# AsherBond/0-kno-vectorx

Measured on AMD Instinct MI355X. Metric: header_range_256 proofs/sec, higher is better.
Workload: dtype u64 (Goldilocks) / u8 (hashes)

## Files before the change

0-kno-vectorx_amd/csrc/vx_bus.hip:

```cpp
#include <string.h>

#include <memory>

#include "vx_bus.h"
#include "vx_table_shapes.h"

int32_t vx_one_table_hook(void*, const uint64_t* pub, size_t n_pub, const uint64_t* cap, size_t cw, uint64_t* chal, size_t n_chal) {
    vx_shared_challenges_n(&pub, &n_pub, &cap, 1, cw, chal, n_chal);
    return VX_OK;
}

int32_t vx_tables_proof_bound(const vx_stark_config* cfg, size_t hdr_words, const TableShape* tables, size_t n_tables, size_t* n_words) {
    size_t total = hdr_words;
    for (size_t k = 0; k < n_tables; ++k) {
        size_t w = 0;
        VX_TRY(vx_stark_proof_bound(tables[k].air_id, cfg, tables[k].log_n, &w));
        total += w;
    }
    *n_words = total;
    return VX_OK;
}
int32_t vx_tables_proof_bound(const vx_stark_config* cfg, size_t hdr_words, std::initializer_list<TableShape> tables, size_t* n_words) {
    return vx_tables_proof_bound(cfg, hdr_words, tables.begin(), tables.size(), n_words);
}
std::array<TableShape, 3> vx_justification_shapes(size_t n_authorities, size_t n_sig) {
    return {{{VX_AIR_SHA_CHAIN, sha_log_n(n_authorities)}, {ed_air_id(n_sig), ed_log_n(n_sig)}, {s512_air_id(n_sig), s512_log_n(n_sig)}}};
}
size_t vx_justification_proof_bound(const vx_stark_config* cfg, size_t n_authorities, int32_t* rc_out) {
    const auto sh = vx_justification_shapes(n_authorities, sig_quorum(n_authorities));
    size_t w = 0;
    *rc_out = vx_tables_proof_bound(cfg, 0, {sh[0], sh[1], sh[2]}, &w);
    return w;
}

static int32_t size_proof(TableJob& j, int air_id, int log_n, const vx_stark_config* cfg) {
    size_t bound = 0;
    VX_TRY(vx_stark_proof_bound(air_id, cfg, log_n, &bound));
    j.proof.resize(bound);
    return VX_OK;
}
int32_t run_table(vx_ctx* c, TableJob& j, int air_id, int log_n, size_t n_cols, size_t n_pub, const vx_stark_config* cfg, const vx_chal_hook* hook, int consume_trace,
                  const TableGen& gen) {
    VX_TRY(size_proof(j, air_id, log_n, cfg));
    vx_buf* trace = nullptr;
    VX_TRY(vx_alloc(c, n_cols << log_n, &trace));
    uint64_t pub[BusMeet::MAX_PUB];
    int32_t r = gen(c, trace, pub);
    if (r == VX_OK) r = vx_stark_prove_impl(c, air_id, cfg, trace->d, trace->n, consume_trace, log_n, pub, n_pub, j.proof.data(), j.proof.size(), &j.len, hook);
    (void)vx_free(c, trace);
    return r;
}
int TableGroup::add(TableSpec s, int bus, bool local) {
    const int k = g.add(bus, local);
    spec[k] = std::move(s);
    hook[k] = {vx_bus_hook, &g.t[k].party};
    return k;
}
int32_t TableGroup::contexts(int here) {
    if (have_contexts) return VX_OK;
    vx_ctx* c = ctx;
    for (int k = 0; k < g.n; ++k)
        if (g.local(k)) job[k].c = k == here ? ctx : (c = c ? vx_side_ctx(c) : nullptr);
    VX_CHECK(c, "%s: no side context for every table (the provers meet at their challenge hooks, each on a context of its own)", what);
    have_contexts = true;
    return VX_OK;
}
int32_t TableGroup::run(int k) {
    const TableSpec& s = spec[k];
    TableJob& j = job[k];
    if (s.gen) return run_table(j.c, j, s.air_id, s.log_n, s.n_cols, s.n_pub, cfg, &hook[k], s.consume_trace, s.gen);
    VX_TRY(size_proof(j, s.air_id, s.log_n, cfg));
    return vx_stark_prove_impl(j.c, s.air_id, cfg, s.trace->d, s.trace->n, s.consume_trace, s.log_n, s.pub, s.n_pub, j.proof.data(), j.proof.size(), &j.len, &hook[k]);
}
int32_t TableGroup::prove(int here, std::vector<int> order) {
    VX_TRY(contexts(here));
    for (int k = 0; k < g.n; ++k)
        if (g.local(k) && k != here) {
            job[k].c->err.clear();
            g.start(k, [this, k] {
                (void)hipSetDevice(job[k].c->device);
                return run(k);
            });
        }
    if (here >= 0) g.run_here(here, [&] { return run(here); });
    g.finish();
    if (order.empty()) {
        if (here >= 0) order.push_back(here);
        for (int k = 0; k < g.n; ++k)
            if (k != here) order.push_back(k);
    }
    int who = -1;
    const int32_t rc = g.first_error(order, &who);
    if (rc == VX_OK || (who >= 0 && who == here)) return rc;
    if (who < 0) return vx_fail(ctx, rc, "%s: %s", what, BusGroup::ALL_RELEASED);
    const char* msg = vx_last_error(job[who].c);
    if (!msg[0]) return vx_fail(ctx, rc, "%s: the %s table failed", what, spec[who].name);
    if (strncmp(msg, what, strlen(what)) == 0) return vx_fail(ctx, rc, "%s", msg);
    return vx_fail(ctx, rc, "%s: %s", what, msg);
}
int32_t pack_blob(vx_ctx* ctx, const char* what, uint64_t magic, const uint64_t* request, size_t n_request, const TableJob* const* jobs, size_t n_jobs, uint64_t* blob_out, size_t blob_cap,
                  size_t* blob_len) {
    size_t total = 1 + n_request + n_jobs;
    for (size_t k = 0; k < n_jobs; ++k) total += jobs[k]->len;
    *blob_len = total;
    if (!blob_out || blob_cap < total) return vx_fail(ctx, VX_ERR_BUFSZ, "%s: the blob needs %zu words, buffer has %zu", what, total, blob_cap);
    uint64_t* w = blob_out;
    *w++ = magic;
    for (size_t k = 0; k < n_request; ++k) *w++ = request[k];
    for (size_t k = 0; k < n_jobs; ++k) *w++ = jobs[k]->len;
    for (size_t k = 0; k < n_jobs; ++k) memcpy(w, jobs[k]->proof.data(), jobs[k]->len * 8), w += jobs[k]->len;
    return VX_OK;
}
int32_t pack_blob(vx_ctx* ctx, const char* what, uint64_t magic, std::initializer_list<uint64_t> request, std::initializer_list<const TableJob*> jobs, uint64_t* blob_out,
                  size_t blob_cap, size_t* blob_len) {
    return pack_blob(ctx, what, magic, request.begin(), request.size(), jobs.begin(), jobs.size(), blob_out, blob_cap, blob_len);
}

int vx_justification_add(TableGroup& g, const vx_justification* just, std::function<int32_t(vx_ctx*)> pre, int bus, unsigned mask) {
    const size_t n_auth = just->num_authorities;
    auto chosen = std::make_shared<std::vector<uint8_t>>(n_auth, 0);
    size_t n_sig = 0;
    for (size_t i = 0; i < n_auth && n_sig < sig_quorum(n_auth); ++i)
        if (just->validator_signed[i]) (*chosen)[i] = 1, ++n_sig;
    const auto sh = vx_justification_shapes(n_auth, n_sig);
    const int sl = sh[0].log_n, el = sh[1].log_n, hl = sh[2].log_n;
    const int first = g.add({"authority-set commitment", sh[0].air_id, sl, VX_SHA_AIR_COLS, 10, 0,
                             [=](vx_ctx* c, vx_buf* st, uint64_t* spub) {
                                 if (pre) VX_TRY(pre(c));
                                 uint8_t com[32];
                                 VX_TRY(vx_sha_chain_trace_dev(c, just->pubkeys, n_auth, chosen->data(), 1, sl, st->d, spub, com));
                                 if (memcmp(com, just->authority_set_hash, 32) != 0) return vx_fail(c, VX_ERR_STATEMENT, "authority-set commitment mismatch");
                                 return (int32_t)VX_OK;
                             }},
                            bus, mask & 1);
    g.add({"Ed25519", sh[1].air_id, el, VX_ED_AIR_COLS, 2, 0,
           [=](vx_ctx* c, vx_buf* et, uint64_t* epub) { return vx_ed_trace_dev(c, just->pubkeys, just->signatures, just->precommit, 53, chosen->data(), n_auth, el, 1, et->d, epub); }},
          bus, mask >> 1 & 1);
    g.add({"SHA-512", sh[2].air_id, hl, VX_SHA512_AIR_COLS, 15, 0,
           [=](vx_ctx* c, vx_buf* ht, uint64_t* hpub) { return vx_sha512_trace_dev(c, just->pubkeys, just->signatures, just->precommit, chosen->data(), n_auth, hl, 1, ht->d, hpub); }},
          bus, mask >> 2 & 1);
    return first;
}
```

0-kno-vectorx_amd/csrc/vx_core.hip:

```cpp
#include <stdarg.h>
#include <stdlib.h>
#include <stdio.h>

#include "gl.cuh"
#include <dlfcn.h>

#include "vx_internal.h"

__attribute__((constructor)) static void vx_runtime_env() { setenv("GPU_MAX_HW_QUEUES", "16", 0); }

int32_t vx_fail(vx_ctx* ctx, int32_t code, const char* fmt, ...) {
    char buf[512];
    va_list ap;
    va_start(ap, fmt);
    vsnprintf(buf, sizeof buf, fmt, ap);
    va_end(ap);
    if (ctx) ctx->err = buf;
    return code;
}

static int32_t make_powtab(vx_ctx* ctx, uint64_t base, PowTab* out) {
    std::vector<uint64_t> h(3 * 2048);
    uint64_t b = base;
    for (int l = 0; l < 3; ++l) {
        uint64_t acc = 1;
        for (int j = 0; j < 2048; ++j) {
            h[l * 2048 + j] = acc;
            acc = glh::mul(acc, b);
        }
        b = glh::pow(b, 2048);
    }
    VX_HIP(hipMalloc(&out->d, h.size() * 8));
    VX_HIP(hipMemcpyAsync(out->d, h.data(), h.size() * 8, hipMemcpyHostToDevice, ctx->stream));
    VX_HIP(hipStreamSynchronize(ctx->stream));
    return VX_OK;
}

int32_t vx_get_shift_tab(vx_ctx* ctx, uint64_t base, PowTab* out) {
    auto it = ctx->shift_tabs.find(base);
    if (it == ctx->shift_tabs.end()) {
        PowTab t;
        VX_TRY(make_powtab(ctx, base, &t));
        it = ctx->shift_tabs.emplace(base, t).first;
    }
    *out = it->second;
    return VX_OK;
}

int32_t vx_get_tw2(vx_ctx* ctx, int log_s, int inverse, Tw2* out) {
    const int lo_bits = (log_s + 1) / 2, hi_bits = log_s - lo_bits;
    const int key = log_s * 2 + (inverse ? 1 : 0);
    auto it = ctx->tw2.find(key);
    if (it == ctx->tw2.end()) {
        const size_t nlo = (size_t)1 << lo_bits, nhi = (size_t)1 << hi_bits;
        std::vector<uint64_t> h(nlo + nhi);
        uint64_t w = glh::root(log_s);
        if (inverse) w = glh::inv(w);
        uint64_t acc = 1;
        for (size_t j = 0; j < nlo; ++j) {
            h[j] = acc;
            acc = glh::mul(acc, w);
        }
        const uint64_t wh = acc;
        acc = 1;
        for (size_t j = 0; j < nhi; ++j) {
            h[nlo + j] = acc;
            acc = glh::mul(acc, wh);
        }
        uint64_t* d = nullptr;
        VX_HIP(hipMalloc(&d, h.size() * 8));
        VX_HIP(hipMemcpyAsync(d, h.data(), h.size() * 8, hipMemcpyHostToDevice, ctx->stream));
        VX_HIP(hipStreamSynchronize(ctx->stream));
        it = ctx->tw2.emplace(key, d).first;
    }
    out->lo = it->second;
    out->hi = it->second + ((size_t)1 << lo_bits);
    out->lo_bits = lo_bits;
    return VX_OK;
}

void vx_pool_trim(vx_ctx* ctx) {
    (void)hipStreamSynchronize(ctx->stream);
    for (auto& kv : ctx->pool_free)
        for (void* p : kv.second) (void)hipFree(p);
    ctx->pool_free.clear();
}
void* vx_pool_alloc(vx_ctx* ctx, size_t bytes) {
    const size_t gran = (size_t)2 << 20;
    const size_t sz = ((bytes ? bytes : 1) + gran - 1) / gran * gran;
    auto it = ctx->pool_free.find(sz);
    void* p = nullptr;
    if (it != ctx->pool_free.end() && !it->second.empty()) {
        p = it->second.back();
        it->second.pop_back();
    } else if (hipMalloc(&p, sz) != hipSuccess) {
        (void)hipGetLastError();
        vx_pool_trim(ctx);
        if (hipMalloc(&p, sz) != hipSuccess) {
            (void)hipGetLastError();
            return nullptr;
        }
    }
    ctx->pool_live[p] = sz;
    return p;
}
void vx_pool_free(vx_ctx* ctx, void* p) {
    if (!p) return;
    auto it = ctx->pool_live.find(p);
    if (it == ctx->pool_live.end()) {
        (void)hipFree(p);
        return;
    }
    ctx->pool_free[it->second].push_back(p);
    ctx->pool_live.erase(it);
}

int32_t vx_scratch(vx_ctx* ctx, size_t n, uint64_t** out) {
    if (ctx->scratch_n < n) {
        if (ctx->scratch) {
            vx_pool_free(ctx, ctx->scratch);
            ctx->scratch = nullptr;
            ctx->scratch_n = 0;
        }
        ctx->scratch = (uint64_t*)vx_pool_alloc(ctx, n * 8);
        if (!ctx->scratch) return vx_fail(ctx, VX_ERR_OOM, "scratch: cannot allocate %zu bytes", n * 8);
        ctx->scratch_n = n;
    }
    *out = ctx->scratch;
    return VX_OK;
}

extern "C" {

const char* vx_backend_name(void) { return "hip-gfx950"; }

static thread_local int g_side_ctx = 0;
int32_t vx_ctx_create(int device, vx_ctx** out) {
    if (!out) return VX_ERR_ARG;
    *out = nullptr;
    int n_dev = 0;
    if (hipGetDeviceCount(&n_dev) != hipSuccess || n_dev == 0 || device < 0 || device >= n_dev) return VX_ERR_DEVICE;
    vx_ctx* ctx = new vx_ctx();
    ctx->device = device;
    ctx->scratch = nullptr;
    ctx->scratch_n = 0;
    ctx->pinned = nullptr;
    ctx->pinned_n = 0;
    {
        const char* sm = getenv("VX_SYNC_MODE");
        const char m = sm ? sm[0] : 'b';
        (void)hipSetDevice(device);
        (void)hipSetDeviceFlags(m == 's' ? hipDeviceScheduleSpin : m == 'y' ? hipDeviceScheduleYield : hipDeviceScheduleBlockingSync);
        (void)hipGetLastError();
    }
    hipError_t se = hipSetDevice(device);
    if (se == hipSuccess) {
        const char* sp = getenv("VX_STREAM_PRIO");
        int least = 0, greatest = 0;
        if (sp && sp[0] == '1' && hipDeviceGetStreamPriorityRange(&least, &greatest) == hipSuccess && least != greatest)
            se = hipStreamCreateWithPriority(&ctx->stream, hipStreamDefault, g_side_ctx ? least : greatest);
        else se = hipStreamCreate(&ctx->stream);
    }
    if (se != hipSuccess ||
        hipEventCreate(&ctx->ev0) != hipSuccess || hipEventCreate(&ctx->ev1) != hipSuccess) {
        delete ctx;
        return VX_ERR_DEVICE;
    }
    int32_t rc = make_powtab(ctx, glh::ROOT_2_32, &ctx->tw_fwd);
    if (rc == VX_OK) rc = make_powtab(ctx, glh::inv(glh::ROOT_2_32), &ctx->tw_inv);
    if (rc == VX_OK) {
        std::vector<uint64_t> f(2048), b(2048);
        uint64_t w = glh::root(12), wi = glh::inv(w), a = 1, c = 1;
        for (int j = 0; j < 2048; ++j) {
            f[j] = a;
            b[j] = c;
            a = glh::mul(a, w);
            c = glh::mul(c, wi);
        }
        if (hipMalloc(&ctx->w12_fwd, 2048 * 8) != hipSuccess || hipMalloc(&ctx->w12_inv, 2048 * 8) != hipSuccess ||
            hipMemcpy(ctx->w12_fwd, f.data(), 2048 * 8, hipMemcpyHostToDevice) != hipSuccess ||
            hipMemcpy(ctx->w12_inv, b.data(), 2048 * 8, hipMemcpyHostToDevice) != hipSuccess)
            rc = VX_ERR_DEVICE;
    }
    if (rc == VX_OK) {
        ctx->pinned_n = 1 << 20;
        if (hipHostMalloc(&ctx->pinned, ctx->pinned_n) != hipSuccess) rc = VX_ERR_DEVICE;
    }
    if (rc != VX_OK) {
        delete ctx;
        return rc;
    }
    *out = ctx;
    return VX_OK;
}

int32_t vx_ctx_destroy(vx_ctx* ctx) {
    if (!ctx) return VX_ERR_ARG;
    if (ctx->side) {
        vx_ctx_destroy(ctx->side);
        ctx->side = nullptr;
    }
    hipSetDevice(ctx->device);
    hipStreamSynchronize(ctx->stream);
    for (auto& kv : ctx->shift_tabs) hipFree(kv.second.d);
    for (auto& kv : ctx->periodic_cache) hipFree(kv.second);
    for (auto& kv : ctx->tw2) hipFree(kv.second);
    hipFree(ctx->tw_fwd.d);
    hipFree(ctx->tw_inv.d);
    hipFree(ctx->w12_fwd);
    hipFree(ctx->w12_inv);
    if (ctx->scratch) vx_pool_free(ctx, ctx->scratch);
    vx_pool_trim(ctx);
    for (auto& kv : ctx->pool_live) hipFree(kv.first);
    if (ctx->pinned) hipHostFree(ctx->pinned);
    hipEventDestroy(ctx->ev0);
    hipEventDestroy(ctx->ev1);
    hipStreamDestroy(ctx->stream);
    delete ctx;
    return VX_OK;
}

int32_t vx_sync(vx_ctx* ctx) {
    if (!ctx) return VX_ERR_ARG;
    VX_HIP(hipStreamSynchronize(ctx->stream));
    return VX_OK;
}
const char* vx_last_error(const vx_ctx* ctx) { return ctx ? ctx->err.c_str() : "null ctx"; }

int32_t vx_timer_start(vx_ctx* ctx) {
    if (!ctx) return VX_ERR_ARG;
    VX_HIP(hipEventRecord(ctx->ev0, ctx->stream));
    return VX_OK;
}
int32_t vx_timer_stop(vx_ctx* ctx, float* ms) {
    if (!ctx || !ms) return VX_ERR_ARG;
    VX_HIP(hipEventRecord(ctx->ev1, ctx->stream));
    VX_HIP(hipEventSynchronize(ctx->ev1));
    VX_HIP(hipEventElapsedTime(ms, ctx->ev0, ctx->ev1));
    return VX_OK;
}

int32_t vx_alloc(vx_ctx* ctx, size_t n, vx_buf** out) {
    if (!ctx || !out) return VX_ERR_ARG;
    VX_CHECK(n > 0, "vx_alloc: n == 0");
    vx_buf* b = new vx_buf{nullptr, n};
    b->d = (uint64_t*)vx_pool_alloc(ctx, n * 8);
    if (!b->d) {
        delete b;
        return vx_fail(ctx, VX_ERR_OOM, "device allocation of %zu bytes failed", n * 8);
    }
    *out = b;
    return VX_OK;
}
int32_t vx_free(vx_ctx* ctx, vx_buf* buf) {
    if (!ctx || !buf) return VX_ERR_ARG;
    vx_pool_free(ctx, buf->d);
    delete buf;
    return VX_OK;
}
int32_t vx_upload(vx_ctx* ctx, vx_buf* dst, size_t off, const uint64_t* src, size_t n) {
    if (!ctx || !dst || !src) return VX_ERR_ARG;
    VX_CHECK(off + n <= dst->n, "vx_upload: range [%zu,%zu) exceeds buffer of %zu", off, off + n, dst->n);
    VX_HIP(hipMemcpyAsync(dst->d + off, src, n * 8, hipMemcpyHostToDevice, ctx->stream));
    VX_HIP(hipStreamSynchronize(ctx->stream));
    return VX_OK;
}
int32_t vx_download(vx_ctx* ctx, const vx_buf* src, size_t off, uint64_t* dst, size_t n) {
    if (!ctx || !dst || !src) return VX_ERR_ARG;
    VX_CHECK(off + n <= src->n, "vx_download: range [%zu,%zu) exceeds buffer of %zu", off, off + n, src->n);
    VX_HIP(hipMemcpyAsync(dst, src->d + off, n * 8, hipMemcpyDeviceToHost, ctx->stream));
    VX_HIP(hipStreamSynchronize(ctx->stream));
    return VX_OK;
}
int32_t vx_copy(vx_ctx* ctx, vx_buf* dst, size_t doff, const vx_buf* src, size_t soff, size_t n) {
    if (!ctx || !dst || !src) return VX_ERR_ARG;
    VX_CHECK(doff + n <= dst->n && soff + n <= src->n, "vx_copy: out of range");
    VX_HIP(hipMemcpyAsync(dst->d + doff, src->d + soff, n * 8, hipMemcpyDeviceToDevice, ctx->stream));
    return VX_OK;
}
void* vx_buf_devptr(const vx_buf* buf) { return buf ? buf->d : nullptr; }
size_t vx_buf_len(const vx_buf* buf) { return buf ? buf->n : 0; }
}

__global__ void k_fill_random(uint64_t* d, size_t n, uint64_t seed) {
    size_t i = blockIdx.x * (size_t)blockDim.x + threadIdx.x;
    size_t stride = (size_t)gridDim.x * blockDim.x;
    for (; i < n; i += stride) {
        uint64_t z = seed + 0x9E3779B97F4A7C15ULL * (i + 1);
        z = (z ^ (z >> 30)) * 0xBF58476D1CE4E5B9ULL;
        z = (z ^ (z >> 27)) * 0x94D049BB133111EBULL;
        z ^= z >> 31;
        d[i] = gl_canon(z);
    }
}
template <int OP>
__global__ void k_batch(const uint64_t* a, const uint64_t* b, uint64_t* o, size_t n) {
    size_t i = blockIdx.x * (size_t)blockDim.x + threadIdx.x;
    size_t stride = (size_t)gridDim.x * blockDim.x;
    for (; i < n; i += stride) {
        uint64_t x = a[i], y = OP == 3 ? 0 : b[i], r;
        if (OP == 0) r = gl_add(x, y);
        else if (OP == 1) r = gl_sub(x, y);
        else if (OP == 2) r = gl_mul(x, y);
        else r = x ? gl_inv(x) : 0;
        o[i] = r;
    }
}
__global__ void k_ext_mul(const uint64_t* a, const uint64_t* b, uint64_t* o, size_t n) {
    size_t i = blockIdx.x * (size_t)blockDim.x + threadIdx.x;
    size_t stride = (size_t)gridDim.x * blockDim.x;
    for (; i < n; i += stride) {
        gl2 x{a[2 * i], a[2 * i + 1]}, y{b[2 * i], b[2 * i + 1]};
        gl2 r = gl2_mul(x, y);
        o[2 * i] = r.a;
        o[2 * i + 1] = r.b;
    }
}
static inline unsigned grid_for(size_t n) {
    size_t g = (n + 255) / 256;
    return (unsigned)(g < 1 ? 1 : (g > 2048 ? 2048 : g));
}
template <int OP>
static int32_t batch_op(vx_ctx* ctx, const vx_buf* a, const vx_buf* b, vx_buf* o, size_t n) {
    if (!ctx || !a || !o || (OP != 3 && !b)) return VX_ERR_ARG;
    VX_CHECK(n <= a->n && n <= o->n && (OP == 3 || n <= b->n), "batch op: n exceeds a buffer");
    if (n == 0) return VX_OK;
    hipLaunchKernelGGL(k_batch<OP>, dim3(grid_for(n)), dim3(256), 0, ctx->stream, a->d, OP == 3 ? a->d : b->d, o->d, n);
    VX_HIP(hipGetLastError());
    return VX_OK;
}
extern "C" {
int32_t vx_fill_random(vx_ctx* ctx, vx_buf* dst, size_t off, size_t n, uint64_t seed) {
    if (!ctx || !dst) return VX_ERR_ARG;
    VX_CHECK(off + n <= dst->n, "vx_fill_random: out of range");
    if (n == 0) return VX_OK;
    hipLaunchKernelGGL(k_fill_random, dim3(grid_for(n)), dim3(256), 0, ctx->stream, dst->d + off, n, seed);
    VX_HIP(hipGetLastError());
    return VX_OK;
}
int32_t vx_field_batch_add(vx_ctx* c, const vx_buf* a, const vx_buf* b, vx_buf* o, size_t n) { return batch_op<0>(c, a, b, o, n); }
int32_t vx_field_batch_sub(vx_ctx* c, const vx_buf* a, const vx_buf* b, vx_buf* o, size_t n) { return batch_op<1>(c, a, b, o, n); }
int32_t vx_field_batch_mul(vx_ctx* c, const vx_buf* a, const vx_buf* b, vx_buf* o, size_t n) { return batch_op<2>(c, a, b, o, n); }
int32_t vx_field_batch_inv(vx_ctx* c, const vx_buf* a, vx_buf* o, size_t n) { return batch_op<3>(c, a, nullptr, o, n); }
int32_t vx_ext_batch_mul(vx_ctx* ctx, const vx_buf* a, const vx_buf* b, vx_buf* o, size_t n) {
    if (!ctx || !a || !b || !o) return VX_ERR_ARG;
    VX_CHECK(2 * n <= a->n && 2 * n <= b->n && 2 * n <= o->n, "ext batch mul: n exceeds a buffer");
    if (n == 0) return VX_OK;
    hipLaunchKernelGGL(k_ext_mul, dim3(grid_for(n)), dim3(256), 0, ctx->stream, a->d, b->d, o->d, n);
    VX_HIP(hipGetLastError());
    return VX_OK;
}

int32_t vx_gather_proofs(vx_ctx* ctx, void* nccl_comm, int world, const uint64_t* mine, size_t n_words, uint64_t* out) {
    if (!ctx || !nccl_comm || !mine || !out || world < 1) return VX_ERR_ARG;
    typedef int (*all_gather_fn)(const void*, void*, size_t, int, void*, hipStream_t);
    static all_gather_fn all_gather = nullptr;
    if (!all_gather) all_gather = (all_gather_fn)dlsym(RTLD_DEFAULT, "ncclAllGather");
    if (!all_gather) {
        for (const char* name : {"librccl.so.1", "librccl.so"}) {
            void* h = dlopen(name, RTLD_NOLOAD | RTLD_LAZY);
            if (h && (all_gather = (all_gather_fn)dlsym(h, "ncclAllGather"))) break;
        }
    }
    if (!all_gather) return vx_fail(ctx, VX_ERR_DEVICE, "gather: ncclAllGather is not loaded in this process");
    if (n_words == 0) return VX_OK;
    uint64_t* sc;
    VX_TRY(vx_scratch(ctx, n_words * ((size_t)world + 1), &sc));
    VX_HIP(hipMemcpyAsync(sc, mine, n_words * 8, hipMemcpyHostToDevice, ctx->stream));
    const int rc = all_gather(sc, sc + n_words, n_words, 5, nccl_comm, ctx->stream);
    if (rc != 0) return vx_fail(ctx, VX_ERR_DEVICE, "gather: ncclAllGather failed (%d)", rc);
    VX_HIP(hipMemcpyAsync(out, sc + n_words, n_words * 8 * (size_t)world, hipMemcpyDeviceToHost, ctx->stream));
    VX_HIP(hipStreamSynchronize(ctx->stream));
    return VX_OK;
}
}

vx_ctx* vx_side_ctx(vx_ctx* ctx) {
    if (!ctx->side) {
        g_side_ctx = 1;
        if (vx_ctx_create(ctx->device, &ctx->side) != VX_OK) ctx->side = nullptr;
        g_side_ctx = 0;
    }
    return ctx->side;
}
```

0-kno-vectorx_amd/csrc/vx_internal.h:

```cpp
#pragma once
#include <hip/hip_runtime.h>
#include <stdint.h>
#include <map>
#include <string>
#include <vector>

#pragma GCC visibility push(default)
#include "../../include/vx.h"
#pragma GCC visibility pop
#include "glh.h"

#ifndef VX_TAIL_PRIO
#define VX_TAIL_PRIO 1
#endif
#if VX_TAIL_PRIO
#define VX_TAIL_KERNEL_ENTRY() __builtin_amdgcn_s_setprio(3)
#else
#define VX_TAIL_KERNEL_ENTRY() ((void)0)
#endif

struct vx_buf {
    uint64_t* d;
    size_t n;
};

struct PowTab {
    uint64_t* d;
};

struct vx_ctx {
    int device;
    hipStream_t stream;
    hipEvent_t ev0, ev1;
    std::string err;
    PowTab tw_fwd, tw_inv;
    uint64_t *w12_fwd, *w12_inv;
    std::map<uint64_t, PowTab> shift_tabs;
    std::map<int, uint64_t*> tw2;
    uint64_t* scratch;
    size_t scratch_n;
    void* pinned;
    size_t pinned_n;
    std::map<size_t, std::vector<void*>> pool_free;
    std::map<void*, size_t> pool_live;
    vx_ctx* side = nullptr;
    std::map<uint64_t, uint64_t*> periodic_cache;
};
vx_ctx* vx_side_ctx(vx_ctx* ctx);
void* vx_pool_alloc(vx_ctx* ctx, size_t bytes);
void vx_pool_free(vx_ctx* ctx, void* p);
void vx_pool_trim(vx_ctx* ctx);
int32_t vx_fail(vx_ctx* ctx, int32_t code, const char* fmt, ...);

struct Scratch {
    vx_ctx* ctx = nullptr;
    uint64_t* base = nullptr;
    size_t words = 0;
    hipError_t err = hipSuccess;
    std::vector<std::pair<uint64_t**, size_t>> regions;
    Scratch() = default;
    Scratch(const Scratch&) = delete;
    Scratch& operator=(const Scratch&) = delete;
    ~Scratch() {
        if (base) vx_pool_free(ctx, base);
    }
    void add(uint64_t*& p, size_t n) { regions.push_back({&p, words}), words += n; }
    void alloc(vx_ctx* c) {
        ctx = c, base = (uint64_t*)vx_pool_alloc(c, words * 8);
        for (auto& r : regions) *r.first = base ? base + r.second : nullptr;
    }
    bool ok() const { return base && err == hipSuccess; }
    void keep(hipError_t e) {
        if (err == hipSuccess) err = e;
    }
    void copy(void* dst, const void* src, size_t bytes, hipMemcpyKind kind) {
        if (ok()) err = hipMemcpyAsync(dst, src, bytes, kind, ctx->stream);
    }
    void up(void* dst, const void* src, size_t bytes) { copy(dst, src, bytes, hipMemcpyHostToDevice); }
    void down(void* dst, const void* src, size_t bytes) { copy(dst, src, bytes, hipMemcpyDeviceToHost); }
    void fill(void* dst, int byte, size_t bytes) {
        if (ok()) err = hipMemsetAsync(dst, byte, bytes, ctx->stream);
    }
    void launched() { keep(hipGetLastError()); }
    void sync() {
        if (ok()) err = hipStreamSynchronize(ctx->stream);
    }
    int32_t status(const char* what) const {
        if (!base) return vx_fail(ctx, VX_ERR_OOM, "%s: out of device memory", what);
        return err == hipSuccess ? VX_OK : vx_fail(ctx, VX_ERR_DEVICE, "%s: %s", what, hipGetErrorString(err));
    }
};

struct vx_tree {
    uint64_t* levels;
    size_t n_leaves;
    int cap_height;
    size_t total;
};

#define VX_HIP(call)                                                                              \
    do {                                                                                          \
        hipError_t e_ = (call);                                                                   \
        if (e_ != hipSuccess)                                                                     \
            return vx_fail(ctx, e_ == hipErrorOutOfMemory ? VX_ERR_OOM : VX_ERR_DEVICE, "%s: %s", \
                           #call, hipGetErrorString(e_));                                         \
    } while (0)
#define VX_CHECK(cond, ...)                                   \
    do {                                                      \
        if (!(cond)) return vx_fail(ctx, VX_ERR_ARG, __VA_ARGS__); \
    } while (0)
#define VX_TRY(call)            \
    do {                        \
        int32_t r_ = (call);    \
        if (r_ != VX_OK) return r_; \
    } while (0)

int32_t vx_get_shift_tab(vx_ctx* ctx, uint64_t base, PowTab* out);
int32_t vx_scratch(vx_ctx* ctx, size_t n_u64, uint64_t** out);
int32_t vx_merkle_build_dev(vx_ctx* ctx, const uint64_t* data, size_t n_leaves, size_t leaf_len, int layout,
                            int cap_height, vx_tree** out);

int32_t vx_ntt_dev(vx_ctx* ctx, uint64_t* d, int log_n, size_t n_cols, size_t col_stride, int inverse, uint64_t shift, int order);
int32_t vx_lde_dev(vx_ctx* ctx, const uint64_t* src, int log_n, size_t n_cols, int rate_bits, uint64_t shift, int src_kind,
                   uint64_t* dst, uint64_t* coeffs_out);
int32_t vx_gather_rows_dev(vx_ctx* ctx, const uint64_t* lde, int log_N, size_t n_cols, const uint64_t* leaf_idx, size_t n_idx,
                           uint64_t* out);
void vx_gather_rows_enqueue(vx_ctx* ctx, const uint64_t* lde, int log_N, size_t n_cols, const uint64_t* idx_d, size_t n_idx, uint64_t* out_d);
void vx_merkle_open_enqueue(vx_ctx* ctx, const vx_tree* tree, const uint64_t* idx_d, size_t n_idx, uint64_t* out_d);
void vx_fri_leaves_enqueue(vx_ctx* ctx, const uint64_t* evals, int log_n, int arity_bits, const uint64_t* idx_d, size_t n_idx, uint64_t* out_d);
int32_t vx_fri_fold_dev(vx_ctx* ctx, const uint64_t* evals, int log_n, int arity_bits, const uint64_t beta[2], uint64_t shift,
                        uint64_t* out);
int32_t vx_fri_layer_tree_dev(vx_ctx* ctx, const uint64_t* evals, int log_n, int arity_bits, int cap_height, vx_tree** out);
int32_t vx_fri_leaves_dev(vx_ctx* ctx, const uint64_t* evals, int log_n, int arity_bits, const uint64_t* leaf_idx, size_t n_idx,
                          uint64_t* out);

struct Tw2 {
    const uint64_t* lo;
    const uint64_t* hi;
    int lo_bits;
};
int32_t vx_get_tw2(vx_ctx* ctx, int log_s, int inverse, Tw2* out);
int32_t vx_lde_consume_dev(vx_ctx* ctx, uint64_t* values, int log_n, size_t n_cols, int rate_bits, uint64_t shift, uint64_t* dst);
struct vx_chal_hook {
    int32_t (*fn)(void* user, const uint64_t* pub, size_t n_pub, const uint64_t* cap, size_t cap_words, uint64_t* chal, size_t n_chal);
    void* user;
};
int32_t vx_stark_prove_impl(vx_ctx* ctx, int air_id, const vx_stark_config* cfg, uint64_t* trace_d, size_t trace_len, int consume_trace,
                            int log_n, const uint64_t* public_inputs, size_t n_public, uint64_t* proof_out, size_t proof_cap,
                            size_t* proof_len, const vx_chal_hook* hook = nullptr);
void vx_shared_challenges_n(const uint64_t* const* pubs, const size_t* n_pubs, const uint64_t* const* caps, size_t k, size_t cap_words, uint64_t* out, size_t n_out);
void vx_shared_challenges(const uint64_t* pub_a, size_t n_a, const uint64_t* cap_a, const uint64_t* pub_b, size_t n_b, const uint64_t* cap_b,
                          size_t cap_words, uint64_t* out, size_t n_out);
int32_t vx_stark_verify_ext(const vx_stark_config* cfg, const uint64_t* proof, size_t proof_len, int expect_air, const uint64_t* expect_public,
                            size_t n_expect_public, const uint64_t* ext_chal, const uint64_t** apub_out, int* log_n_out, char* err, size_t errlen);
int32_t vx_lde_keep_dev(vx_ctx* ctx, const uint64_t* values, int log_n, size_t n_cols, int rate_bits, uint64_t shift, uint64_t* coef_brev,
                        uint64_t* dst);
int32_t vx_scan_cols_dev(vx_ctx* ctx, uint64_t* data, int log_n, size_t n_cols, uint64_t* totals_host);
int32_t vx_sha_tree_trace_dev(vx_ctx* ctx, const uint8_t* state_roots, const uint8_t* data_roots, size_t n_leaves, int log_tree, uint64_t* trace_d,
                              uint64_t pub_out[17]);
int32_t vx_bus_close_dev(vx_ctx* ctx, uint64_t* z_cols, int log_n, uint64_t aux_pub[2]);
int32_t vx_ed_trace_dev(vx_ctx* ctx, const uint8_t* pubkeys, const uint8_t* sigs, const uint8_t* msg, uint32_t msg_len, const uint8_t* signed_flags, size_t n_sigs,
                        int log_n, uint64_t bus_on, uint64_t* trace_d, uint64_t pub_out[2]);
int32_t vx_sha512_trace_dev(vx_ctx* ctx, const uint8_t* pubkeys, const uint8_t* sigs, const uint8_t* msg, const uint8_t* flags, size_t n_sigs, int log_n, uint64_t bus_on,
                            uint64_t* trace_d, uint64_t pub_out[15]);
int32_t vx_epoch_end_trace_dev(vx_ctx* ctx, const uint8_t* header_d, size_t header_bytes, uint32_t start_position, uint32_t num_authorities, uint64_t bus_on, uint64_t* trace_d,
                               uint64_t pub_out[10], uint32_t* window_length_out);
int32_t vx_sha_chain_trace_dev(vx_ctx* ctx, const uint8_t* pubkeys, size_t n_keys, const uint8_t* signed_flags, uint64_t bus_on, int log_n, uint64_t* trace_d,
                               uint64_t public_inputs_out[10], uint8_t commitment_out[32]);
int32_t vx_merkle_open_trace_dev(vx_ctx* ctx, const vx_tree* tree, const uint64_t* leaf_idx, size_t n_idx, int log_n, uint64_t* trace_d, uint64_t pub_out[9]);
void vx_merkle_levels_launch(vx_ctx* ctx, uint64_t* levels, size_t n_leaves, size_t cap);
```

Measured before the change: 8.541.

## Plan how table-prover contexts map onto shared or own HIP streams

Side contexts now start on their parent's stream. TableGroup::contexts then gives each local table a stream using a plan based on VX_TABLE_STREAMS, GPU_MAX_HW_QUEUES and the number of live host contexts, and can optionally share streams. The aim is to avoid oversubscribing hardware queues when several provers or tables run at once on one device. With default settings each non-caller table still gets its own stream, so behaviour should stay close to before. The change adds a stream synchronize and a small bind copy during setup.

Result: slower. 8.435 (-1.2%).

```diff
diff --git a/0-kno-vectorx_amd/csrc/vx_bus.hip b/0-kno-vectorx_amd/csrc/vx_bus.hip
--- a/0-kno-vectorx_amd/csrc/vx_bus.hip
+++ b/0-kno-vectorx_amd/csrc/vx_bus.hip
@@ -3,6 +3,7 @@
 #include <memory>
 
 #include "vx_bus.h"
+#include "vx_stream_plan.h"
 #include "vx_table_shapes.h"
 
 int32_t vx_one_table_hook(void*, const uint64_t* pub, size_t n_pub, const uint64_t* cap, size_t cw, uint64_t* chal, size_t n_chal) {
@@ -59,9 +60,23 @@
 int32_t TableGroup::contexts(int here) {
     if (have_contexts) return VX_OK;
     vx_ctx* c = ctx;
+    int n_local = 0;
     for (int k = 0; k < g.n; ++k)
-        if (g.local(k)) job[k].c = k == here ? ctx : (c = c ? vx_side_ctx(c) : nullptr);
+        if (g.local(k)) job[k].c = k == here ? ctx : (c = c ? vx_side_ctx(c) : nullptr), ++n_local;
     VX_CHECK(c, "%s: no side context for every table (the provers meet at their challenge hooks, each on a context of its own)", what);
+    const bool caller_busy = here >= 0 && g.local(here);
+    const int K = vx_plan_streams(getenv("VX_TABLE_STREAMS"), vx_plan_queues(getenv("GPU_MAX_HW_QUEUES")), vx_ctxs_alive(ctx->device), n_local);
+    hipStream_t streams[BusGroup::MAX] = {ctx->stream};
+    int i = 0;
+    for (int k = 0; k < g.n; ++k)
+        if (g.local(k) && k != here) {
+            const int j = vx_plan_deal(i, K, caller_busy);
+            if (j > 0 && !streams[j]) streams[j] = vx_ctx_own_stream(job[k].c);
+            VX_CHECK(streams[j], "%s: no stream for the %s table", what, spec[k].name);
+            const int32_t r = vx_ctx_use_stream(job[k].c, streams[j]);
+            if (r != VX_OK) return vx_fail(ctx, r, "%s: %s", what, vx_last_error(job[k].c));
+            ++i;
+        }
     have_contexts = true;
     return VX_OK;
 }
diff --git a/0-kno-vectorx_amd/csrc/vx_core.hip b/0-kno-vectorx_amd/csrc/vx_core.hip
--- a/0-kno-vectorx_amd/csrc/vx_core.hip
+++ b/0-kno-vectorx_amd/csrc/vx_core.hip
@@ -1,6 +1,8 @@
 #include <stdarg.h>
 #include <stdlib.h>
 #include <stdio.h>
+
+#include <atomic>
 
 #include "gl.cuh"
 #include <dlfcn.h>
@@ -134,7 +136,16 @@
 
 const char* vx_backend_name(void) { return "hip-gfx950"; }
 
-static thread_local int g_side_ctx = 0;
+static hipError_t make_stream(hipStream_t* s, bool side) {
+    const char* sp = getenv("VX_STREAM_PRIO");
+    int least = 0, greatest = 0;
+    if (sp && sp[0] == '1' && hipDeviceGetStreamPriorityRange(&least, &greatest) == hipSuccess && least != greatest)
+        return hipStreamCreateWithPriority(s, hipStreamDefault, side ? least : greatest);
+    return hipStreamCreate(s);
+}
+static thread_local vx_ctx* g_side_of = nullptr;
+static std::atomic<int> g_host_ctxs[64];
+static std::atomic<int>& host_ctxs(int device) { return g_host_ctxs[device < 0 ? 0 : device > 63 ? 63 : device]; }
 int32_t vx_ctx_create(int device, vx_ctx** out) {
     if (!out) return VX_ERR_ARG;
     *out = nullptr;
@@ -155,14 +166,12 @@
     }
     hipError_t se = hipSetDevice(device);
     if (se == hipSuccess) {
-        const char* sp = getenv("VX_STREAM_PRIO");
-        int least = 0, greatest = 0;
-        if (sp && sp[0] == '1' && hipDeviceGetStreamPriorityRange(&least, &greatest) == hipSuccess && least != greatest)
-            se = hipStreamCreateWithPriority(&ctx->stream, hipStreamDefault, g_side_ctx ? least : greatest);
-        else se = hipStreamCreate(&ctx->stream);
+        if (g_side_of) ctx->stream = g_side_of->stream;
+        else if ((se = make_stream(&ctx->own, false)) == hipSuccess) ctx->stream = ctx->own;
     }
     if (se != hipSuccess ||
         hipEventCreate(&ctx->ev0) != hipSuccess || hipEventCreate(&ctx->ev1) != hipSuccess) {
+        if (ctx->own) (void)hipStreamDestroy(ctx->own);
         delete ctx;
         return VX_ERR_DEVICE;
     }
@@ -190,6 +199,7 @@
         delete ctx;
         return rc;
     }
+    if (!g_side_of) ctx->host_made = true, ++host_ctxs(device);
     *out = ctx;
     return VX_OK;
 }
@@ -215,7 +225,8 @@
     if (ctx->pinned) hipHostFree(ctx->pinned);
     hipEventDestroy(ctx->ev0);
     hipEventDestroy(ctx->ev1);
-    hipStreamDestroy(ctx->stream);
+    if (ctx->own) hipStreamDestroy(ctx->own);
+    if (ctx->host_made) --host_ctxs(ctx->device);
     delete ctx;
     return VX_OK;
 }
@@ -377,9 +388,28 @@
 
 vx_ctx* vx_side_ctx(vx_ctx* ctx) {
     if (!ctx->side) {
-        g_side_ctx = 1;
+        g_side_of = ctx;
         if (vx_ctx_create(ctx->device, &ctx->side) != VX_OK) ctx->side = nullptr;
-        g_side_ctx = 0;
+        g_side_of = nullptr;
     }
     return ctx->side;
 }
+hipStream_t vx_ctx_own_stream(vx_ctx* ctx) {
+    if (!ctx->own && (hipSetDevice(ctx->device) != hipSuccess || make_stream(&ctx->own, true) != hipSuccess)) {
+        (void)hipGetLastError();
+        ctx->own = nullptr;
+    } else if (ctx->own && !ctx->own_bound) {
+        ctx->own_bound = true;
+        if (hipMemcpyAsync(ctx->pinned, ctx->w12_fwd, 8, hipMemcpyDeviceToHost, ctx->own) != hipSuccess || hipStreamSynchronize(ctx->own) != hipSuccess)
+            (void)hipGetLastError();
+    }
+    return ctx->own;
+}
+int32_t vx_ctx_use_stream(vx_ctx* ctx, hipStream_t s) {
+    if (ctx->host_made || !s) return vx_fail(ctx, VX_ERR_ARG, "a context made by the host keeps its stream, and a side context needs one");
+    if (ctx->stream == s) return VX_OK;
+    VX_HIP(hipStreamSynchronize(ctx->stream));
+    ctx->stream = s;
+    return VX_OK;
+}
+int vx_ctxs_alive(int device) { return host_ctxs(device).load(); }
diff --git a/0-kno-vectorx_amd/csrc/vx_internal.h b/0-kno-vectorx_amd/csrc/vx_internal.h
--- a/0-kno-vectorx_amd/csrc/vx_internal.h
+++ b/0-kno-vectorx_amd/csrc/vx_internal.h
@@ -31,6 +31,9 @@
 struct vx_ctx {
     int device;
     hipStream_t stream;
+    hipStream_t own = nullptr;
+    bool own_bound = false;
+    bool host_made = false;
     hipEvent_t ev0, ev1;
     std::string err;
     PowTab tw_fwd, tw_inv;
@@ -47,6 +50,9 @@
     std::map<uint64_t, uint64_t*> periodic_cache;
 };
 vx_ctx* vx_side_ctx(vx_ctx* ctx);
+hipStream_t vx_ctx_own_stream(vx_ctx* ctx);
+int32_t vx_ctx_use_stream(vx_ctx* ctx, hipStream_t s);
+int vx_ctxs_alive(int device);
 void* vx_pool_alloc(vx_ctx* ctx, size_t bytes);
 void vx_pool_free(vx_ctx* ctx, void* p);
 void vx_pool_trim(vx_ctx* ctx);
diff --git a/0-kno-vectorx_amd/csrc/vx_stream_plan.h b/0-kno-vectorx_amd/csrc/vx_stream_plan.h
--- /dev/null
+++ b/0-kno-vectorx_amd/csrc/vx_stream_plan.h
@@ -0,0 +1,43 @@
+#pragma once
+#include <stdlib.h>
+#include <string.h>
+
+static const int VX_DEFAULT_HW_QUEUES = 4;
+
+inline int vx_plan_share(int queues, int alive, int tables) {
+    if (tables < 1) return 1;
+    if (queues < 1) queues = 1;
+    if (alive < 1) alive = 1;
+    if ((long long)queues >= (long long)alive * tables) return tables;
+    const int k = queues / alive;
+    return k < 1 ? 1 : k;
+}
+
+inline bool vx_plan_number(const char* s, int* out) {
+    if (!s || !*s) return false;
+    int v = 0, digits = 0;
+    for (; *s; ++s, ++digits) {
+        if (*s < '0' || *s > '9' || digits == 9) return false;
+        v = v * 10 + (*s - '0');
+    }
+    *out = v;
+    return true;
+}
+
+inline int vx_plan_queues(const char* value) {
+    int q = 0;
+    return vx_plan_number(value, &q) && q >= 1 ? q : VX_DEFAULT_HW_QUEUES;
+}
+
+inline int vx_plan_streams(const char* value, int queues, int alive, int tables) {
+    if (tables < 1) return 1;
+    int k = 0;
+    if (value && strcmp(value, "share") == 0) return vx_plan_share(queues, alive, tables);
+    if (!vx_plan_number(value, &k)) return tables;
+    return k < 1 ? 1 : k > tables ? tables : k;
+}
+
+inline int vx_plan_deal(int i, int k, bool caller_busy) {
+    if (k <= 1) return 0;
+    return caller_busy ? 1 + i % (k - 1) : i % k;
+}
```
